# benabbouosama/DEEPL-Project

Measured on AMD Instinct MI355X. Metric: images/sec train step, TransVAE-Large f16d32 256px bs256, higher is better.
Workload: dtype bf16

## Files before the change

deepl-project_amd/csrc/conv3x3_halo.hip:

```cpp
#include "igemm_common.h"

namespace {

template <int BM, int BN, int WGM, int WGN, int BST, int EPI>
__global__ __launch_bounds__(WGM* WGN * 64) void conv3x3_halo_kernel(const IgemmArgs p) {
    constexpr int BK = 64, NW = WGM * WGN, TW = 16, TH = BM / TW, HWD = TW + 2, HP = (TH + 2) * HWD;
    constexpr int A_PIECES = (HP * 8 + 63) / 64;
    constexpr int WTM = BM / WGM, WTN = BN / WGN, MF = WTM / 16, NF = WTN / 16;
    constexpr bool PIPE_ALL = (MF + NF) * 4 * (BK / 32) <= (NW == 4 && BM == 256 ? 128 : 80);
    constexpr int A_IT = (A_PIECES + NW - 1) / NW;
    constexpr int A_BYTES = A_PIECES * 1024, B_BYTES = BN * BK * 2;
    constexpr int B_INSTR = BN / 8, B_IT = B_INSTR / NW;
    static_assert(BST == 2 || BST == 3, "weight ring depth");
    static_assert(B_INSTR % NW == 0 && WTM % 16 == 0 && WTN % 16 == 0, "tile shape");

    extern __shared__ __attribute__((aligned(16))) char smem[];
    TV_PROBE_DECL
    char* const a_buf = smem;
    char* const b_buf = smem + 2 * A_BYTES;

    const int tid = threadIdx.x;
    const int lane = tid & 63;
    const int wave = __builtin_amdgcn_readfirstlane(tid >> 6);
    const int wm = wave / WGN, wn = wave % WGN;
    int tile_n, tile_m;
    if (p.xcd_order) {
        const int lin = blockIdx.x, j = lin >> 3;
        tile_n = j % p.tiles_n;
        tile_m = (j / p.tiles_n) * 8 + (lin & 7);
        if (tile_m >= p.tiles_m) return;
    } else {
        tile_n = blockIdx.x % p.tiles_n;
        tile_m = blockIdx.x / p.tiles_n;
    }
    const int n0 = tile_n * BN;
    const int tiles_x = p.w_out / TW, tiles_y = p.h_out / TH;
    const int b = tile_m / (tiles_x * tiles_y);
    const int trem = tile_m - b * (tiles_x * tiles_y);
    const int y0 = (trem / tiles_x) * TH, x0 = (trem % tiles_x) * TW;

    const int a_c16 = ((lane & 7) ^ ((lane >> 3) & 7)) * 16;
    auto a_voff_of = [&](int j) {
        int l8 = lane >> 3;
        asm volatile("" : "+v"(l8));
        const int hp = j * 8 + l8;
        const int hy = hp / HWD, hx = hp - hy * HWD;
        const int iy = y0 - 1 + hy, ix = x0 - 1 + hx;
        const bool ok = hp < HP && (unsigned)iy < (unsigned)p.h_in && (unsigned)ix < (unsigned)p.w_in;
        return ok ? ((b * p.h_in + iy) * p.w_in + ix) * p.ldx * 2 + a_c16 : OOB_OFFSET;
    };
    auto b_voff_of = [&](int j) {
        int l8 = lane >> 3;
        asm volatile("" : "+v"(l8));
        const int row = j * 8 + l8;
        const int rl = row % WTN;
        const int fr = bfrag_reader(rl);
        const int c = ((lane & 7) ^ swz_of<BK>(fr)) * 8;
        const int n = n0 + row;
        return (n < p.N) ? (n * p.K + c) * 2 : OOB_OFFSET;
    };
#ifdef TV_ABL_K1
    const int cch = 1;
#else
    const int cch = p.c_in / BK;
#endif

    constexpr bool VOFF_REGS = MF * NF * 4 + (MF + NF) * 8 <= 160 || BST == 3 || !PIPE_ALL;
    int a_voff_r[VOFF_REGS ? A_IT : 1], b_voff_r[VOFF_REGS ? B_IT : 1];
    if constexpr (VOFF_REGS) {
#pragma unroll
        for (int it = 0; it < A_IT; ++it) a_voff_r[it] = a_voff_of(it * NW + wave);
#pragma unroll
// ... 61 lines not shown
                        acc[i][j] = __builtin_amdgcn_mfma_f32_16x16x32_bf16(bfr[kk][j], af[kk][i], acc[i][j], 0, 0, 0);
                        const int idx = (kk * MF + i) * NF + j;
                        if (idx % GAP == GAP - 1 && idx / GAP < NIH) {
                            __builtin_amdgcn_sched_barrier(0);
                            issue(idx / GAP);
                            __builtin_amdgcn_sched_barrier(0);
                        }
                    }
        } else {
#pragma unroll
            for (int kk = 0; kk < BK / 32; ++kk) {
                bf16x8 af[MF], bfr[NF];
#pragma unroll
                for (int i = 0; i < MF; ++i) af[i] = *(const bf16x8*)(abase + a_off[i] + (((kk * 4 + fq) ^ a_sw[i]) << 4));
                const int coff = ((kk * 4 + fq) ^ sw) * 16;
#pragma unroll
                for (int j = 0; j < NF; ++j) bfr[j] = *(const bf16x8*)(bbase + b_row_off + bfrag_off(j) * (BK * 2) + coff);
#pragma unroll
                for (int i = 0; i < MF; ++i)
#pragma unroll
                    for (int j = 0; j < NF; ++j) {
                        acc[i][j] = __builtin_amdgcn_mfma_f32_16x16x32_bf16(bfr[j], af[i], acc[i][j], 0, 0, 0);
                        const int idx = (kk * MF + i) * NF + j;
                        if (idx % GAP == GAP - 1 && idx / GAP < NIH) {
                            __builtin_amdgcn_sched_barrier(0);
                            issue(idx / GAP);
                            __builtin_amdgcn_sched_barrier(0);
                        }
                    }
            }
        }
    };

    constexpr bool PP = NW == 8 && PIPE_ALL && BST == 3;
    if constexpr (PP) {
        constexpr int ATAPS = 6, A_PT = (A_IT + ATAPS - 1) / ATAPS;
        static_assert(A_PT == 1, "one halo piece per wave and tap");
        constexpr auto nsure = [](int tap) { return (tap >= 0 && tap < ATAPS && tap < A_IT && (tap + 1) * NW <= A_PIECES) ? 1 : 0; };
        const int grp = wave >> 2;
        bf16x8 fa[2][MF], fb[2][NF];
#pragma unroll
        for (int it = 0; it < A_IT; ++it) issue_a(a_buf, it, 0);
        issue_b(b_buf, 0, 0);
        issue_b(b_buf + B_BYTES, 1, 0);
        wait_vmcnt<0>();
        if (grp == 1) __builtin_amdgcn_s_barrier();
        int bcur = 0;
        for (int ch = 0; ch < cch; ++ch) {
            const char* acur = a_buf + (ch & 1) * A_BYTES;
            char* anxt = a_buf + ((ch + 1) & 1) * A_BYTES;
            const bool more = ch + 1 < cch;
            static_for<9>([&](auto tap_c) {
                constexpr int tap = decltype(tap_c)::value;
                constexpr int toff = (tap / 3) * HWD + (tap % 3);
                const char* const bslot = b_buf + bcur * B_BYTES;
                char* const bfill = b_buf + ((bcur + 2 >= BST) ? bcur + 2 - BST : bcur + 2) * B_BYTES;
                const bool b_go = (tap + 2 < 9) || more;
                const int b_koff = ((tap + 2 < 9) ? (tap + 2) * p.c_in + ch * BK : (tap + 2 - 9) * p.c_in + (ch + 1) * BK) * 2;
                auto load_dma = [&]() {
                    if (b_go) {
#pragma unroll
                        for (int it = 0; it < B_IT; ++it) issue_b_piece(bfill, it, b_koff);
                    }
                    if (tap < ATAPS && tap < A_IT && more) issue_a(anxt, tap, ch + 1);
                };
                __builtin_amdgcn_s_barrier();
                TV_T(1);
                int hpb = hp_base;
                asm volatile("" : "+v"(hpb));
#ifndef TV_ABL_NO_LDSREAD
#pragma unroll
                for (int kk = 0; kk < 2; ++kk) {
#pragma unroll
                    for (int i = 0; i < MF; ++i) {
                        const int hp = hpb + i * HWD + toff;
                        fa[kk][i] = *(const bf16x8*)(acur + hp * (BK * 2) + (((kk * 4 + fq) ^ (hp & 7)) << 4));
                    }
                    const int coff = ((kk * 4 + fq) ^ sw) * 16;
#pragma unroll
                    for (int j = 0; j < NF; ++j) fb[kk][j] = *(const bf16x8*)(bslot + b_row_off + bfrag_off(j) * (BK * 2) + coff);
                }
#else
                if (tap == 0 && ch == 0) {
                    for (int kk = 0; kk < 2; ++kk) {
                        for (int i = 0; i < MF; ++i) { fa[kk][i] = bf16x8{1, 1, 1, 1, 1, 1, 1, 1}; asm volatile("" : "+v"(fa[kk][i])); }
                        for (int j = 0; j < NF; ++j) { fb[kk][j] = bf16x8{1, 1, 1, 1, 1, 1, 1, 1}; asm volatile("" : "+v"(fb[kk][j])); }
                    }
                }
#endif
                __builtin_amdgcn_sched_barrier(0);
                TV_T(3);
                load_dma();
                __builtin_amdgcn_sched_barrier(0);
                TV_T(2);
                asm volatile("s_waitcnt lgkmcnt(0)" ::: "memory");
                if (more) wait_vmcnt<nsure(tap - 1) + B_IT + nsure(tap)>();
                else if (tap + 2 < 9) wait_vmcnt<B_IT>();
                else wait_vmcnt<0>();
                TV_T(0);
                __builtin_amdgcn_s_barrier();
                TV_T(5);
                __builtin_amdgcn_s_setprio(1);
#pragma unroll
                for (int kk = 0; kk < 2; ++kk)
#pragma unroll
                    for (int i = 0; i < MF; ++i)
#pragma unroll
                        for (int j = 0; j < NF; ++j) acc[i][j] = __builtin_amdgcn_mfma_f32_16x16x32_bf16(fb[kk][j], fa[kk][i], acc[i][j], 0, 0, 0);
                __builtin_amdgcn_s_setprio(0);
                __builtin_amdgcn_sched_barrier(0);
                TV_T(4);
                bcur = (bcur + 1 == BST) ? 0 : bcur + 1;
            });
        }
        if (grp == 0) __builtin_amdgcn_s_barrier();
    } else if constexpr (PIPE_ALL) {
        constexpr int ATAPS = 6, A_PT = (A_IT + ATAPS - 1) / ATAPS;
        constexpr auto nsure = [](int tap) {
            int n = 0;
            for (int it = tap * A_PT; it < tap * A_PT + A_PT; ++it)
                if (tap >= 0 && tap < ATAPS && it < A_IT && (it + 1) * NW <= A_PIECES) ++n;
            return n;
        };
        constexpr int HMF = MF * NF, NIS = B_IT + A_PT, HGAP = HMF / NIS;
        static_assert(HGAP >= 1, "more DMA pieces than MFMAs in a half-step");
        bf16x8 f0a[MF], f0b[NF], f1a[MF], f1b[NF];
#ifdef TV_ABL_CHEAP_ADDR
        const int abl_a_off = (hp_base & ~7) * (BK * 2) + fi * (BK * 2) + ((fq ^ (fi & 7)) << 4);
#endif
#ifdef TV_ABL_NO_LDSREAD
        for (int i = 0; i < MF; ++i) { f0a[i] = bf16x8{1, 1, 1, 1, 1, 1, 1, 1}; f1a[i] = f0a[i]; asm volatile("" : "+v"(f0a[i]), "+v"(f1a[i])); }
        for (int j = 0; j < NF; ++j) { f0b[j] = bf16x8{1, 1, 1, 1, 1, 1, 1, 1}; f1b[j] = f0b[j]; asm volatile("" : "+v"(f0b[j]), "+v"(f1b[j])); }
#endif
        auto read_half = [&](const char* abase, const char* bbase, int toff, int kk, bf16x8 (&fa)[MF], bf16x8 (&fb)[NF]) {
#ifdef TV_ABL_NO_LDSREAD
            return;
#endif
            int hpb = hp_base;
            asm volatile("" : "+v"(hpb));
#pragma unroll
            for (int i = 0; i < MF; ++i) {
#ifdef TV_ABL_CHEAP_ADDR
                fa[i] = *(const bf16x8*)(abase + abl_a_off + i * HWD * (BK * 2) + kk * 64);
#else
                const int hp = hpb + i * HWD + toff;
                fa[i] = *(const bf16x8*)(abase + hp * (BK * 2) + (((kk * 4 + fq) ^ (hp & 7)) << 4));
#endif
            }
// ... 144 lines not shown
    __builtin_amdgcn_s_setprio(0);
    TV_T(5);
#ifdef TV_ABL_NO_EPI
    {
        float chk = 0.f;
#pragma unroll
        for (int i = 0; i < MF; ++i)
#pragma unroll
            for (int j = 0; j < NF; ++j) chk += acc[i][j][0] + acc[i][j][1] + acc[i][j][2] + acc[i][j][3];
        if (chk != 123.456f) return;
    }
#endif
    f32x4 bvals[NF];
    load_bias<WTN>(p, lane, n0 + wn * WTN, bvals);
    const int pix0 = (b * p.h_out + y0 + wm * MF) * p.w_out + x0;
    epilogue<WTM, WTN, EPI, true>(p, acc, bvals, smem, wave, lane, n0 + wn * WTN, [&](int r) { return pix0 + (r >> 4) * p.w_out + (r & 15); });
    TV_T(6);
    TV_PROBE_DUMP(wave, lane);
}

template <int BM, int BN, int WGM, int WGN, int BST>
int launch_halo_one(const IgemmArgs& a_in, hipStream_t s) {
    constexpr int NW = WGM * WGN, HP = (BM / 16 + 2) * 18;
    constexpr int RING = 2 * (((HP * 8 + 63) / 64) * 1024) + BST * BN * 64 * 2;
    constexpr int EPI = epilogue_lds_bytes<BM / WGM, BN / WGN>(NW);
    constexpr int BYTES = RING > EPI ? RING : EPI;
    if constexpr (BYTES > LDS_MAX) {
        return -1;
    } else {
        const int tiles_m = a_in.batch * (a_in.h_out / (BM / 16)) * (a_in.w_out / 16);
        IgemmArgs a = a_in;
        a.tiles_m = tiles_m;
        a.xcd_order = (g_xcd_order && a.tiles_n > 1) ? 1 : 0;
        dim3 grid((unsigned)(a.xcd_order ? 8 * a.tiles_n * ((tiles_m + 7) / 8) : tiles_m * a.tiles_n)), block(NW * 64);
        auto go = [&](auto epi) {
            constexpr int EPI_MODE = decltype(epi)::value;
            static TvPerDeviceOnce attr_once;
            if (attr_once.first()) {
                (void)hipFuncSetAttribute((const void*)conv3x3_halo_kernel<BM, BN, WGM, WGN, BST, EPI_MODE>, hipFuncAttributeMaxDynamicSharedMemorySize, BYTES);
            }
            hipLaunchKernelGGL((conv3x3_halo_kernel<BM, BN, WGM, WGN, BST, EPI_MODE>), grid, block, BYTES, s, a);
        };
        const int epi = epilogue_mode(a);
        if (epi == 1) go(std::integral_constant<int, 1>{});
        else if (epi == 2) go(std::integral_constant<int, 2>{});
        else go(std::integral_constant<int, 0>{});
        return 0;
    }
}

template <int BM, int BN, int WGM, int WGN>
int launch_halo_ring(const IgemmArgs& a, int ring, hipStream_t s) {
    if (ring >= 3 && launch_halo_one<BM, BN, WGM, WGN, 3>(a, s) == 0) return 0;
    return launch_halo_one<BM, BN, WGM, WGN, 2>(a, s);
}

int launch_halo_impl(IgemmArgs& a, hipStream_t s) {
    if (!(a.kh == 3 && a.kw == 3 && a.stride == 1 && a.pad == 1 && a.up_shift == 0 && a.dil_mask == 0 && !a.shuffle)) return -1;
    if (a.c_in % 64 != 0 || a.N <= 64 || a.x_bytes == 0 || a.w_bytes == 0) return -1;
    if (a.h_in != a.h_out || a.w_in != a.w_out || a.w_out % 16 != 0 || a.h_out % 8 != 0) return -1;
    const int N = a.N;
    const bool h16 = a.h_out % 16 == 0;
    int bm = 128;
    int bn = pick_tile(a.M, N, h16, h16 && (N == 192 || N % 128 != 0), &bm);
    if (N % 192 == 0 && h16 && g_cfg_bn == 0 && g_halo_ring == 3 && !g_halo_w4) { bn = 192; bm = 256; }
    if (g_cfg_bn == 256 && N % 256 == 0 && h16) { bn = 256; bm = 256; }
    else if (g_cfg_bn == 192 && N % 192 == 0 && h16) { bn = 192; bm = 256; }
    else if (g_cfg_bn == 128) { bn = (N % 192 == 0 && N % 128 != 0) ? 192 : 128; bm = 128; }
    if (g_cfg_bm) bm = g_cfg_bm;
    if (bm == 256 && !h16) bm = 128;
    if (bn == 192) {
        a.tiles_n = N / 192;
        if (bm == 256 && g_halo_w4) return launch_halo_ring<256, 192, 2, 2>(a, (g_halo_ring == 3 && a.tiles_n == 1) || g_halo_ring == 4 ? 3 : 2, s);
        if (bm == 256) return launch_halo_ring<256, 192, 4, 2>(a, (g_halo_ring == 3 || g_halo_ring == 4) ? 3 : 2, s);
        return launch_halo_ring<128, 192, 2, 2>(a, g_halo_ring == 4 ? 3 : 2, s);
    }
// ... 18 lines not shown
```

deepl-project_amd/csrc/igemm_common.h:

```cpp
#pragma once
#pragma clang fp contract(off)
#include "common.h"

#include <type_traits>

namespace tvi {

struct IgemmArgs {
    const bf16* x;
    const bf16* w;
    const float* bias;
    const bf16* res;
    const bf16* aux;
    bf16* pre;
    bf16* out;
    const char* zeros;
    int M, N, K;
    int batch, h_in, w_in, c_in, ldx;
    int h_out, w_out, ldo;
    int kh, kw, stride, pad, up_shift, dil_mask;
    int tiles_n, tiles_m, xcd_order;
    int sup_r, sup_c;
    int tpb, nchunks;
    int shuffle;
    int act;
    int aux_act;
    int pre_deriv;
    int form;
    const float* rope;
    int rope_tokens, rope_cols;
    int hw_shift, w_shift;
    unsigned dv_hw_m, dv_w_m, dv_cq_m;
    int dv_hw_s, dv_w_s, dv_cq_s;
    int store_nt;
    unsigned out_bytes;
    unsigned x_bytes, w_bytes;
    const bf16* x2;
    unsigned x2_bytes;
    int ldx2, k1_steps;
};

constexpr int LDS_MAX = 160 * 1024;
extern int g_cfg_bm, g_cfg_bn, g_halo_ring;
extern bool g_halo_w4, g_xcd_order, g_epi_modes;
int epilogue_mode(const IgemmArgs& a);
int pick_tile(long long M, int N, bool allow256, bool allow192_256rows, int* bm);
int launch_halo(IgemmArgs& a, hipStream_t s);
#ifdef TV_PROBE
int set_halo_probe(void* dev_buf);
#endif

}

namespace {
using namespace tvi;

#ifndef TV_PIPE_ALL_MAX
#define TV_PIPE_ALL_MAX 80
#endif
#ifndef TV_RD_THREAD
#define TV_RD_THREAD 0
#endif
#ifndef TV_GENERIC_DPHASE
#define TV_GENERIC_DPHASE 1
#endif
#ifndef TV_PERSIST_DRAIN
#define TV_PERSIST_DRAIN 1
#endif

__device__ __forceinline__ constexpr int bfrag_off(int j) { return (j >> 1) * 32 + (j & 1) * 4; }
__device__ __forceinline__ int bfrag_lane_row(int fi) { return (fi >> 2) * 8 + (fi & 3); }
__device__ __forceinline__ int bfrag_reader(int rl) { return (((rl & 31) >> 3) << 2) | (rl & 3); }

__device__ __forceinline__ int fast_div(int x, unsigned m, int sh) {
    return m ? (int)(__umulhi((unsigned)x, m) >> sh) : x;
}
// ... 539 lines not shown
```

deepl-project_amd/csrc/igemm_nt.hip:

```cpp
#include "igemm_common.h"

namespace tvi {
int g_cfg_bm = 0;
int g_cfg_bn = 0;
int g_halo_ring = 3;
bool g_halo_w4 = false;
bool g_xcd_order = true;
int g_supertile = 0;
bool g_epi_modes = true;

int epilogue_mode(const IgemmArgs& a) {
    if (a.rope) return 0;
    if (!g_epi_modes || a.shuffle || a.pre || a.out_bytes == 0) return 0;
    if (a.aux) return (a.aux_act == TV_ACT_DERIV && !a.res) ? 2 : 0;
    return (a.res && a.act == TV_ACT_NONE) ? 1 : 0;
}

int pick_tile(long long M, int N, bool allow256, bool allow192_256rows, int* bm) {
    const long long m256 = (M + 255) / 256, m128 = (M + 127) / 128;
    double best = 1e30;
    int bn = 128;
    *bm = 128;
    auto consider = [&](int cbn, int cbm, long long tiles, double slots, double eff) {
        const double rounds = (double)((long long)((tiles + slots - 1) / slots));
        const double t = rounds * (double)cbm * cbn * (slots / 256.0) / eff;
        if (t < best) { best = t; bn = cbn; *bm = cbm; }
    };
    consider(128, 128, m128 * ((N + 127) / 128), 512.0, 0.85);
    if (N % 192 == 0 && allow192_256rows) consider(192, 256, m256 * (N / 192), 256.0, 0.97);
    if (N % 192 == 0 && N % 128 != 0) consider(192, 128, m128 * (N / 192), 256.0, 0.80);
    if (N % 256 == 0 && allow256) consider(256, 256, m256 * (N / 256), 256.0, 1.0);
    return bn;
}

}

namespace {

// ... 850 lines not shown
    return launch_mode<BK, 1>(a, s);
}

}

extern "C" int tv_set_dma(int on) {
    g_use_dma = on != 0;
    g_addr_mode = (on == 2) ? 1 : 0;
    return 0;
}

extern "C" int tv_set_igemm_halo(int on) {
    g_halo_w4 = on >= 100;
    on %= 100;
    g_xcd_order = on < 10;
    on %= 10;
    g_use_halo = on != 0;
    g_halo_ring = (on == 2) ? 2 : (on == 4 ? 4 : 3);
    return 0;
}

extern "C" int tv_set_igemm_nt_threshold(int mib) {
    g_nt_threshold_mb = mib;
    return 0;
}

extern "C" int tv_set_igemm_persist(int on) {
    if (on == -1) g_loop8 = 0;
    else if (on == -2) g_loop8 = 1;
    else g_persist = on;
    return 0;
}

extern "C" int tv_set_igemm_supertile(int v) {
    g_supertile = v;
    return 0;
}

extern "C" int tv_set_igemm_epilogue(int on) {
    g_epi_modes = on != 0;
    return 0;
}

#ifdef TV_PROBE
extern "C" int tv_set_igemm_probe(void* dev_buf) {
    const bool ok = hipMemcpyToSymbol(HIP_SYMBOL(g_probe_dev), &dev_buf, sizeof(void*)) == hipSuccess;
    return (tvi::set_halo_probe(dev_buf) == 0 && ok) ? 0 : 1;
}
#endif

extern "C" int tv_set_igemm_config(int bm, int bn, int stages, int bk) {
    g_cfg_bm = bm;
    g_cfg_bn = bn;
    g_cfg_stages = stages;
    g_cfg_bk = bk;
    return 0;
}

struct RopeSpec {
    const float* tab;
    int tokens, cols;
};
struct Cat2Spec {
    const void* x2;
    int k1, ldx2;
};
// ... 138 lines not shown
```

deepl-project_amd/transvae/hip/_lib.py:

```python
from __future__ import annotations

import ctypes as C
import glob
import os
import subprocess
import threading

_HERE = os.path.dirname(os.path.abspath(__file__))
PKG_ROOT = os.path.dirname(os.path.dirname(_HERE))
CSRC = os.path.join(PKG_ROOT, "csrc")
SO_PATH = os.environ.get("TV_HIP_SO") or os.path.join(_HERE, "libtransvae_hip.so")

ACT_NONE, ACT_GELU, ACT_SILU = 0, 1, 2
ACT_DERIV, ACT_SAVE_DERIV = 3, 16
ACT_ADD = 4
ACTX_RELU = 5
ACTX_LRELU = 6
GAN_GEN, GAN_BCE, GAN_HINGE, GAN_WGAN = 0, 1, 2, 3
LPIPS_MAP, LPIPS_SIGMOID, LPIPS_CLAMP = 1, 2, 4
POOL3_MAX_S2, POOL3_MAX_S1P1, POOL3_AVG_S1P1 = 0, 1, 2
SSIM_SKIMAGE, SSIM_BOX11 = 0, 1
METRIC_NONE, METRIC_CLIP, METRIC_SIGMOID = 0, 1, 2
IMAGE_NONE, IMAGE_SIGMOID = 0, 1
ERR_UNSUPPORTED = 4
# ... 171 lines not shown
    if r.returncode != 0:
        raise RuntimeError(f"link failed:\n{r.stdout.decode(errors='replace')}")
    return SO_PATH


def load():
    global _lib
    if _lib is not None:
        return _lib
    with _lock:
        if _lib is not None:
            return _lib
        if not os.path.exists(SO_PATH):
            raise RuntimeError(
                f"{SO_PATH} is missing: build it with `python -c 'import __graft_entry__ as g; g.build()'` "
                "(the TransVAE path has no non-HIP fallback)")
        lib = C.CDLL(SO_PATH)
        for name, (res, args) in SIGNATURES.items():
            fn = getattr(lib, name)
            fn.restype = res
            fn.argtypes = args
        lib.tv_set_dma.restype = _I
        lib.tv_set_dma.argtypes = [_I]
        lib.tv_set_igemm_halo.restype = _I
        lib.tv_set_igemm_halo.argtypes = [_I]
        lib.tv_set_igemm_epilogue.restype = _I
        lib.tv_set_igemm_epilogue.argtypes = [_I]
        lib.tv_set_igemm_nt_threshold.restype = _I
        lib.tv_set_igemm_nt_threshold.argtypes = [_I]
        if os.environ.get("TV_IGEMM_NT_MB") is not None:
            lib.tv_set_igemm_nt_threshold(int(os.environ["TV_IGEMM_NT_MB"]))
        lib.tv_set_igemm_persist.restype = _I
        lib.tv_set_igemm_persist.argtypes = [_I]
        lib.tv_set_attn_bwd_mask.restype = _I
        lib.tv_set_attn_bwd_mask.argtypes = [_I]
        lib.tv_set_igemm_config.restype = _I
        lib.tv_set_igemm_config.argtypes = [_I, _I, _I, _I]
        lib.tv_set_wgrad_stages.restype = _I
        lib.tv_set_wgrad_stages.argtypes = [_I]
        lib.tv_set_wgrad_config.restype = _I
        lib.tv_set_wgrad_config.argtypes = [_I, _I, _I]
        lib.tv_set_wgrad_kx3.restype = _I
        lib.tv_set_wgrad_kx3.argtypes = [_I, _I, _I]
        lib.tv_wgrad_tn_which.restype = _I
        lib.tv_wgrad_tn_which.argtypes = [_DP, _I, _I, _I, C.c_char_p, _I]
        if os.environ.get("TV_WGRAD_KX3") is not None:
            lib.tv_set_wgrad_kx3(int(os.environ["TV_WGRAD_KX3"]), 0, 0)
        _lib = lib
    return _lib


def check(rc: int, what: str = "") -> None:
    if rc != 0:
        msg = load().tv_last_error().decode(errors="replace")
        raise RuntimeError(f"libtransvae_hip {what} failed (status {rc}): {msg}")
```

deepl-project_amd/csrc/attention.hip:

```cpp
#include "common.h"

namespace {

#ifndef TV_ATTN_ABL
#define TV_ATTN_ABL 0
#endif
__device__ __forceinline__ f32x16 mfma32(bf16x8 a, bf16x8 b, f32x16 c) {
#if TV_ATTN_ABL & 4
    c[0] += (float)a[0] * (float)b[0];
    return c;
#else
    return __builtin_amdgcn_mfma_f32_32x32x16_bf16(a, b, c, 0, 0, 0);
#endif
}
__device__ __forceinline__ f32x16 mfma32b(bf16x8 a, bf16x8 b, f32x16 c) {
#if TV_ATTN_ABL & 2
    c[0] += (float)a[0] * (float)b[0];
    return c;
#else
    return __builtin_amdgcn_mfma_f32_32x32x16_bf16(a, b, c, 0, 0, 0);
#endif
}
#if TV_ATTN_ABL & 1
__device__ __forceinline__ float fexp2(float x) { return x; }
// ... 635 lines not shown
            const bf16x8 df = pack_acc(s, ss);
#pragma unroll
            for (int db = 0; db < 2; ++db) dqt[db] = mfma32b(kfr[ss][db], df, dqt[db]);
        }
    };
    auto key_block = [&](int t, auto stage_c) {
        constexpr int S = decltype(stage_c)::value;
        if (t + D - 1 < nblk) vm_wait<PIECES * (D - 1)>();
        else vm_wait<0>();
        block_sync();
        half_block(t, stage_c, ic<0>{});
        half_block(t, stage_c, ic<1>{});
    };
    ring_for<NS>(nblk, key_block);
    if (q_ok) {
        bf16* row = p.out + ((size_t)b * p.N + qi) * ld + head * 64;
#pragma unroll
        for (int db = 0; db < 2; ++db)
#pragma unroll
            for (int g = 0; g < 4; ++g) {
                float f[4] = {dqt[db][4 * g] * p.scale, dqt[db][4 * g + 1] * p.scale, dqt[db][4 * g + 2] * p.scale, dqt[db][4 * g + 3] * p.scale};
                if (p.rope) rope_adjoint4(f, p.rope + (size_t)qi * 128, db * 32 + 8 * g + 4 * h);
                bf16x4 v = {(bf16)f[0], (bf16)f[1], (bf16)f[2], (bf16)f[3]};
                attn_store4(row + db * 32 + 8 * g + 4 * h, v);
            }
    }
}

#ifndef TV_ATTN_DKV_QS
#define TV_ATTN_DKV_QS 2
#endif
constexpr int DKV_QS = TV_ATTN_DKV_QS;
constexpr int QT_TILE = DKV_QS * 32 * 128;
constexpr int DKV_STAGE = 2 * QT_TILE + DKV_QS * 256;

__global__ __launch_bounds__(256) void attn_bwd_dkv_kernel(const AttnArgs p) {
    extern __shared__ __attribute__((aligned(16))) char smem[];
    const int lane = threadIdx.x & 63;
    const int wave = __builtin_amdgcn_readfirstlane(threadIdx.x >> 6);
    int tile_x, head, b;
    if (!attn_block(p, tile_x, head, b)) return;
    const int C = p.heads * 64;
    const size_t ld = (size_t)3 * C;
    const bf16* qbase = p.qkv + (size_t)b * p.N * ld + head * 64;
    const bf16* kbase = qbase + C;
    const bf16* vbase = qbase + 2 * C;
    const bf16* gbase = p.d_o + (size_t)b * p.N * C + head * 64;
    const float* del_b = p.delta + ((size_t)b * p.heads + head) * p.N;
    const float* lse_b = del_b + (size_t)p.B * p.heads * p.N;
    const int k0 = tile_x * 128 + wave * 32;
    const int ki = k0 + (lane & 31);
    const int h = lane >> 5;
    const bool k_ok = ki < p.N;

    bf16x8 kf[4], vf[4];
#pragma unroll
    for (int st = 0; st < 4; ++st) {
        bf16x8 a = {0, 0, 0, 0, 0, 0, 0, 0}, v = {0, 0, 0, 0, 0, 0, 0, 0};
        if (k_ok) {
            a = *(const bf16x8*)(kbase + (size_t)ki * ld + 16 * st + 8 * h);
            v = *(const bf16x8*)(vbase + (size_t)ki * ld + 16 * st + 8 * h);
        }
        kf[st] = a;
        vf[st] = v;
    }
    f32x16 dkt[2], dvt[2];
#pragma unroll
    for (int i = 0; i < 16; ++i) dkt[0][i] = dkt[1][i] = dvt[0][i] = dvt[1][i] = 0.f;
    const float c2 = p.scale * 1.4426950408889634f;
    const int ntile = (p.N + 32 * DKV_QS - 1) / (32 * DKV_QS);
    int off_r[4], off_c[2], off_ch[2];
    rows_offsets(lane, off_r);
    cols_offsets<false>(lane, off_c, off_ch);

    int vo_q[DKV_QS], vo_g[DKV_QS];
    stage_offsets<false>(vo_q, (int)ld, wave, lane);
    stage_offsets<false>(vo_g, C, wave, lane);
    const unsigned q_bytes = stage_extent(p.N, (int)ld), g_bytes = stage_extent(p.N, C);
    auto stage = [&](int t, char* sb) {
        stage_rows_buf(sb, qbase, q_bytes, t * 32 * DKV_QS, (int)ld, vo_q, wave);
        stage_rows_buf(sb + QT_TILE, gbase, g_bytes, t * 32 * DKV_QS, C, vo_g, wave);
        if (wave < DKV_QS) {
            const int q = (t * DKV_QS + wave) * 32 + (lane & 31);
            const float* src = (q < p.N) ? ((lane < 32 ? lse_b : del_b) + q) : (const float*)(p.zeros + lane * 4);
            __builtin_amdgcn_global_load_lds(TV_GLB(src), TV_LDS(sb + 2 * QT_TILE + wave * 256), 4, 0, 0);
        }
    };

    const unsigned smem_addr = (unsigned)(uintptr_t)(__attribute__((address_space(3))) char*)smem;
    const char* abs_r[4];
    unsigned abs_c[2], abs_ch[2];
#pragma unroll
    for (int st = 0; st < 4; ++st) abs_r[st] = smem + off_r[st];
#pragma unroll
    for (int db = 0; db < 2; ++db) {
        abs_c[db] = smem_addr + off_c[db];
        abs_ch[db] = smem_addr + off_ch[db];
    }
    const char* abs_st = smem + 16 * h;
    constexpr int NS = TV_ATTN_NS_DKV, D = NS - 1;
#pragma unroll
    for (int i = 0; i < D; ++i)
        if (i < ntile) stage(i, smem + i * DKV_STAGE);
    auto query_tile = [&](int t, auto stage_c, auto sub_c) {
        constexpr int S = decltype(stage_c)::value, U = decltype(sub_c)::value;
        constexpr int QB = S * DKV_STAGE + U * 32 * 128, GB = QB + QT_TILE;
        constexpr int STB = S * DKV_STAGE + 2 * QT_TILE + U * 256;
        f32x16 s, dp;
#pragma unroll
        for (int i = 0; i < 16; ++i) s[i] = 0.f;
        f32x4 nl[4], nd[4];
        nl[0] = *(const f32x4*)(abs_st + STB + 0);
        nl[1] = *(const f32x4*)(abs_st + STB + 32);
        nl[2] = *(const f32x4*)(abs_st + STB + 64);
        nl[3] = *(const f32x4*)(abs_st + STB + 96);
        nd[0] = *(const f32x4*)(abs_st + STB + 128 + 0);
        nd[1] = *(const f32x4*)(abs_st + STB + 128 + 32);
        nd[2] = *(const f32x4*)(abs_st + STB + 128 + 64);
        nd[3] = *(const f32x4*)(abs_st + STB + 128 + 96);
#pragma unroll
        for (int r = 0; r < 16; ++r) dp[r] = nd[r >> 2][r & 3];
        s = mfma32(read_rows_imm<QB>(abs_r[0]), kf[0], s);
        dp = mfma32(read_rows_imm<GB>(abs_r[0]), vf[0], dp);
        s = mfma32(read_rows_imm<QB>(abs_r[1]), kf[1], s);
        dp = mfma32(read_rows_imm<GB>(abs_r[1]), vf[1], dp);
        s = mfma32(read_rows_imm<QB>(abs_r[2]), kf[2], s);
        dp = mfma32(read_rows_imm<GB>(abs_r[2]), vf[2], dp);
        s = mfma32(read_rows_imm<QB>(abs_r[3]), kf[3], s);
        dp = mfma32(read_rows_imm<GB>(abs_r[3]), vf[3], dp);
        if constexpr (U == 0) {
            __builtin_amdgcn_sched_barrier(0);
            if (!(TV_ATTN_ABL & 8) && t + D < ntile) stage(t + D, smem + ((S + D) % NS) * DKV_STAGE);
            __builtin_amdgcn_sched_barrier(0);
        }
        bf16x8 gfr[2][2], qfr[2][2];
#pragma unroll
        for (int db = 0; db < 2; ++db) {
            gfr[0][db] = read_cols_imm<GB>(abs_c[db], abs_ch[db]);
            gfr[1][db] = read_cols_imm<GB + 16 * 128>(abs_c[db], abs_ch[db]);
            qfr[0][db] = read_cols_imm<QB>(abs_c[db], abs_ch[db]);
            qfr[1][db] = read_cols_imm<QB + 16 * 128>(abs_c[db], abs_ch[db]);
        }
#pragma unroll
        for (int r = 0; r < 16; ++r) {
            const float pv = fexp2(fmaf(s[r], c2, nl[r >> 2][r & 3]));
            s[r] = pv;
            dp[r] = pv * dp[r];
        }
        lds_wait_all();
#pragma unroll
        for (int ss = 0; ss < 2; ++ss) {
            const bf16x8 pf = pack_acc(s, ss);
            const bf16x8 df = pack_acc(dp, ss);
#pragma unroll
            for (int db = 0; db < 2; ++db) {
                dvt[db] = mfma32b(gfr[ss][db], pf, dvt[db]);
                dkt[db] = mfma32b(qfr[ss][db], df, dkt[db]);
            }
        }
    };
    auto query_stage = [&](int t, auto stage_c) {
        constexpr int S = decltype(stage_c)::value;
        if (t + D - 1 < ntile) {
            if (wave < DKV_QS) vm_wait<(2 * DKV_QS + 1) * (D - 1)>();
            else vm_wait<2 * DKV_QS * (D - 1)>();
        } else {
            vm_wait<0>();
        }
        block_sync();
        query_tile(t, stage_c, ic<0>{});
        if constexpr (DKV_QS > 1) {
            if ((t * DKV_QS + 1) * 32 < p.N) query_tile(t, stage_c, ic<1>{});
        }
    };
    ring_for<NS>(ntile, query_stage);
    if (k_ok) {
        bf16* krow = p.out + ((size_t)b * p.N + ki) * ld + C + head * 64;
        bf16* vrow = krow + C;
#pragma unroll
        for (int db = 0; db < 2; ++db)
#pragma unroll
            for (int g = 0; g < 4; ++g) {
                float f[4] = {dkt[db][4 * g] * p.scale, dkt[db][4 * g + 1] * p.scale, dkt[db][4 * g + 2] * p.scale, dkt[db][4 * g + 3] * p.scale};
                if (p.rope) rope_adjoint4(f, p.rope + (size_t)ki * 128, db * 32 + 8 * g + 4 * h);
                bf16x4 a = {(bf16)f[0], (bf16)f[1], (bf16)f[2], (bf16)f[3]};
                bf16x4 v = {(bf16)dvt[db][4 * g], (bf16)dvt[db][4 * g + 1], (bf16)dvt[db][4 * g + 2], (bf16)dvt[db][4 * g + 3]};
                attn_store4(krow + db * 32 + 8 * g + 4 * h, a);
                attn_store4(vrow + db * 32 + 8 * g + 4 * h, v);
            }
    }
}

int attn_check(const char* name, int B, int N, int heads, float scale) {
    if (B <= 0 || N <= 0 || heads <= 0 || !(scale > 0.f) || B > 65535 || heads > 65535) {
        tv_set_error("%s: bad shape B=%d N=%d heads=%d scale=%g", name, B, N, heads, (double)scale);
        return TV_ERR_ARG;
    }
    return TV_OK;
}

}

static int g_attn_bwd_mask = 7;
extern "C" int tv_set_attn_bwd_mask(int mask) {
    g_attn_bwd_mask = mask;
// ... 48 lines not shown
```

Before: 160.2.

## Let halo conv3x3 blocks walk several consecutive M tiles with overlapped prefetch

In the pipelined 8-wave halo conv kernel, each block now processes a run of consecutive output tiles (walk) instead of one. The next tile's halo and weight loads are issued during the current tile's last channel chunk, so loads overlap the epilogue, and the vmcnt waits are relaxed to account for the epilogue's outstanding stores. A host heuristic picks walk from tile count versus a 256-slot wave model, and it can be overridden with a new setter. This removes per-block prologue and fill bubbles, at the cost of longer runs that may hurt load balance and of more complex synchronization and register pressure.

```diff
diff --git a/deepl-project_amd/csrc/conv3x3_halo.hip b/deepl-project_amd/csrc/conv3x3_halo.hip
--- a/deepl-project_amd/csrc/conv3x3_halo.hip
+++ b/deepl-project_amd/csrc/conv3x3_halo.hip
@@ -23,21 +23,23 @@
     const int lane = tid & 63;
     const int wave = __builtin_amdgcn_readfirstlane(tid >> 6);
     const int wm = wave / WGN, wn = wave % WGN;
+    constexpr bool PP = NW == 8 && PIPE_ALL && BST == 3;
+    const int walk = PP ? p.walk : 1;
     int tile_n, tile_m;
     if (p.xcd_order) {
         const int lin = blockIdx.x, j = lin >> 3;
         tile_n = j % p.tiles_n;
-        tile_m = (j / p.tiles_n) * 8 + (lin & 7);
+        tile_m = ((j / p.tiles_n) * 8 + (lin & 7)) * walk;
         if (tile_m >= p.tiles_m) return;
     } else {
         tile_n = blockIdx.x % p.tiles_n;
-        tile_m = blockIdx.x / p.tiles_n;
+        tile_m = (blockIdx.x / p.tiles_n) * walk;
     }
     const int n0 = tile_n * BN;
     const int tiles_x = p.w_out / TW, tiles_y = p.h_out / TH;
-    const int b = tile_m / (tiles_x * tiles_y);
+    int b = tile_m / (tiles_x * tiles_y);
     const int trem = tile_m - b * (tiles_x * tiles_y);
-    const int y0 = (trem / tiles_x) * TH, x0 = (trem % tiles_x) * TW;
+    int y0 = (trem / tiles_x) * TH, x0 = (trem % tiles_x) * TW;
 
     const int a_c16 = ((lane & 7) ^ ((lane >> 3) & 7)) * 16;
     auto a_voff_of = [&](int j) {
@@ -165,37 +167,56 @@
         }
     };
 
-    constexpr bool PP = NW == 8 && PIPE_ALL && BST == 3;
     if constexpr (PP) {
         constexpr int ATAPS = 6, A_PT = (A_IT + ATAPS - 1) / ATAPS;
         static_assert(A_PT == 1, "one halo piece per wave and tap");
         constexpr auto nsure = [](int tap) { return (tap >= 0 && tap < ATAPS && tap < A_IT && (tap + 1) * NW <= A_PIECES) ? 1 : 0; };
+        constexpr int NST = MF * (NF / 2);
         const int grp = wave >> 2;
         bf16x8 fa[2][MF], fb[2][NF];
+        const int tile_end = tile_m + walk < p.tiles_m ? tile_m + walk : p.tiles_m;
+        constexpr bool BIAS_RUN = EPI != 0;
+        f32x4 bvals[NF];
+        if constexpr (BIAS_RUN) load_bias<WTN>(p, lane, n0 + wn * WTN, bvals);
 #pragma unroll
         for (int it = 0; it < A_IT; ++it) issue_a(a_buf, it, 0);
         issue_b(b_buf, 0, 0);
         issue_b(b_buf + B_BYTES, 1, 0);
         wait_vmcnt<0>();
         if (grp == 1) __builtin_amdgcn_s_barrier();
-        int bcur = 0;
-        for (int ch = 0; ch < cch; ++ch) {
-            const char* acur = a_buf + (ch & 1) * A_BYTES;
-            char* anxt = a_buf + ((ch + 1) & 1) * A_BYTES;
-            const bool more = ch + 1 < cch;
+        int bcur = 0, apar = 0;
+        int pix0 = (b * p.h_out + y0 + wm * MF) * p.w_out + x0;
+#pragma nounroll
+        for (int ch = 0, tm = tile_m;;) {
+            const bool next = tm + 1 < tile_end, later = tm != tile_m;
+            const char* acur = a_buf + apar * A_BYTES;
+            char* anxt = a_buf + (apar ^ 1) * A_BYTES;
+            apar ^= 1;
+            const bool last = ch + 1 == cch;
+            const bool more = !last || next;
+            const int chn = last ? 0 : ch + 1;
+            if (last && next) {
+                x0 += TW;
+                if (x0 == p.w_out) { x0 = 0; y0 += TH; }
+                if (y0 == p.h_out) { y0 = 0; ++b; }
+                if constexpr (VOFF_REGS) {
+#pragma unroll
+                    for (int it = 0; it < A_IT; ++it) a_voff_r[it] = a_voff_of(it * NW + wave);
+                }
+            }
             static_for<9>([&](auto tap_c) {
                 constexpr int tap = decltype(tap_c)::value;
                 constexpr int toff = (tap / 3) * HWD + (tap % 3);
                 const char* const bslot = b_buf + bcur * B_BYTES;
                 char* const bfill = b_buf + ((bcur + 2 >= BST) ? bcur + 2 - BST : bcur + 2) * B_BYTES;
                 const bool b_go = (tap + 2 < 9) || more;
-                const int b_koff = ((tap + 2 < 9) ? (tap + 2) * p.c_in + ch * BK : (tap + 2 - 9) * p.c_in + (ch + 1) * BK) * 2;
+                const int b_koff = ((tap + 2 < 9) ? (tap + 2) * p.c_in + ch * BK : (tap + 2 - 9) * p.c_in + chn * BK) * 2;
                 auto load_dma = [&]() {
                     if (b_go) {
 #pragma unroll
                         for (int it = 0; it < B_IT; ++it) issue_b_piece(bfill, it, b_koff);
                     }
-                    if (tap < ATAPS && tap < A_IT && more) issue_a(anxt, tap, ch + 1);
+                    if (tap < ATAPS && tap < A_IT && more) issue_a(anxt, tap, chn);
                 };
                 __builtin_amdgcn_s_barrier();
                 TV_T(1);
@@ -227,8 +248,22 @@
                 __builtin_amdgcn_sched_barrier(0);
                 TV_T(2);
                 asm volatile("s_waitcnt lgkmcnt(0)" ::: "memory");
-                if (more) wait_vmcnt<nsure(tap - 1) + B_IT + nsure(tap)>();
-                else if (tap + 2 < 9) wait_vmcnt<B_IT>();
+                auto wait_more = [&](auto base_c) {
+                    constexpr int BASE = decltype(base_c)::value;
+#ifndef TV_ABL_WALK_DRAIN
+                    if constexpr (tap == 0) {
+                        static_assert(BASE + 2 * NST <= 63, "vmcnt is a 6-bit count");
+                        if (ch == 0 && later) {
+                            if (EPI == 0 && (p.form == EF_GELU_D || p.form == EF_SILU_D)) wait_vmcnt<BASE + 2 * NST>();
+                            else wait_vmcnt<BASE + NST>();
+                            return;
+                        }
+                    }
+#endif
+                    wait_vmcnt<BASE>();
+                };
+                if (more) wait_more(std::integral_constant<int, nsure(tap - 1) + B_IT + nsure(tap)>{});
+                else if (tap + 2 < 9) wait_more(std::integral_constant<int, B_IT>{});
                 else wait_vmcnt<0>();
                 TV_T(0);
                 __builtin_amdgcn_s_barrier();
@@ -245,8 +280,44 @@
                 TV_T(4);
                 bcur = (bcur + 1 == BST) ? 0 : bcur + 1;
             });
+            if (!last) {
+                ++ch;
+                continue;
+            }
+            if (grp == 0) __builtin_amdgcn_s_barrier();
+            __builtin_amdgcn_s_setprio(0);
+            TV_T(5);
+            int lane_e = lane;
+            asm volatile("" : "+v"(lane_e));
+            IgemmArgs pe = p;
+            asm volatile("" : "+s"(pe.out), "+s"(pe.pre), "+s"(pe.res), "+s"(pe.aux), "+s"(pe.out_bytes), "+s"(pe.M), "+s"(pe.N), "+s"(pe.ldo),
+                         "+s"(pe.form), "+s"(pe.store_nt), "+s"(pe.bias));
+            if constexpr (!BIAS_RUN) load_bias<WTN>(pe, lane_e, n0 + wn * WTN, bvals);
+#ifdef TV_ABL_NO_EPI
+            float chk = 0.f;
+#pragma unroll
+            for (int i = 0; i < MF; ++i)
+#pragma unroll
+                for (int j = 0; j < NF; ++j) chk += acc[i][j][0] + acc[i][j][1] + acc[i][j][2] + acc[i][j][3];
+            if (chk == 123.456f)
+#endif
+            epilogue<WTM, WTN, EPI, true>(pe, acc, bvals, smem, wave, lane_e, n0 + wn * WTN, [&](int r) { return pix0 + (r >> 4) * p.w_out + (r & 15); });
+            TV_T(6);
+            if (!next) break;
+#pragma unroll
+            for (int i = 0; i < MF; ++i)
+#pragma unroll
+                for (int j = 0; j < NF; ++j) acc[i][j] = f32x4{0.f, 0.f, 0.f, 0.f};
+#ifdef TV_ABL_WALK_DRAIN
+            wait_vmcnt<0>();
+#endif
+            if (grp == 1) __builtin_amdgcn_s_barrier();
+            ch = 0;
+            ++tm;
+            pix0 = (b * p.h_out + y0 + wm * MF) * p.w_out + x0;
         }
-        if (grp == 0) __builtin_amdgcn_s_barrier();
+        TV_PROBE_DUMP(wave, lane);
+        return;
     } else if constexpr (PIPE_ALL) {
         constexpr int ATAPS = 6, A_PT = (A_IT + ATAPS - 1) / ATAPS;
         constexpr auto nsure = [](int tap) {
@@ -457,7 +528,30 @@
         IgemmArgs a = a_in;
         a.tiles_m = tiles_m;
         a.xcd_order = (g_xcd_order && a.tiles_n > 1) ? 1 : 0;
-        dim3 grid((unsigned)(a.xcd_order ? 8 * a.tiles_n * ((tiles_m + 7) / 8) : tiles_m * a.tiles_n)), block(NW * 64);
+        const int epi = epilogue_mode(a);
+        a.walk = 1;
+        constexpr bool WALK_OK = BM == 256 && BN == 192 && NW == 8 && BST == 3;
+        auto direct_form = [](int f) {
+            switch (f) {
+                case EF_PLAIN: case EF_GELU_D: case EF_SILU_D: case EF_GELU: case EF_SILU: case EF_RES_DERIV: case EF_RES2:
+                case EF_RELU: case EF_RELU_MASK: case EF_LRELU: case EF_LRELU_MASK: return true;
+                default: return false;
+            }
+        };
+        if (WALK_OK && g_halo_walk != 1 && (epi != 0 || direct_form(a.form))) {
+            if (g_halo_walk > 1) {
+                a.walk = g_halo_walk < tiles_m ? g_halo_walk : tiles_m;
+            } else {
+                long long best = 0;
+                for (int w = 1; w <= 16; w *= 2) {
+                    const long long runs = (long long)((tiles_m + w - 1) / w) * a.tiles_n;
+                    const long long cost = ((runs + 255) / 256) * (12 * w + 1);
+                    if (w == 1 || cost < best) { best = cost; a.walk = w; }
+                }
+            }
+        }
+        const int runs_m = (tiles_m + a.walk - 1) / a.walk;
+        dim3 grid((unsigned)(a.xcd_order ? 8 * a.tiles_n * ((runs_m + 7) / 8) : runs_m * a.tiles_n)), block(NW * 64);
         auto go = [&](auto epi) {
             constexpr int EPI_MODE = decltype(epi)::value;
             static TvPerDeviceOnce attr_once;
@@ -466,7 +560,6 @@
             }
             hipLaunchKernelGGL((conv3x3_halo_kernel<BM, BN, WGM, WGN, BST, EPI_MODE>), grid, block, BYTES, s, a);
         };
-        const int epi = epilogue_mode(a);
         if (epi == 1) go(std::integral_constant<int, 1>{});
         else if (epi == 2) go(std::integral_constant<int, 2>{});
         else go(std::integral_constant<int, 0>{});
diff --git a/deepl-project_amd/csrc/igemm_common.h b/deepl-project_amd/csrc/igemm_common.h
--- a/deepl-project_amd/csrc/igemm_common.h
+++ b/deepl-project_amd/csrc/igemm_common.h
@@ -22,6 +22,7 @@
     int tiles_n, tiles_m, xcd_order;
     int sup_r, sup_c;
     int tpb, nchunks;
+    int walk;
     int shuffle;
     int act;
     int aux_act;
@@ -41,7 +42,7 @@
 };
 
 constexpr int LDS_MAX = 160 * 1024;
-extern int g_cfg_bm, g_cfg_bn, g_halo_ring;
+extern int g_cfg_bm, g_cfg_bn, g_halo_ring, g_halo_walk;
 extern bool g_halo_w4, g_xcd_order, g_epi_modes;
 int epilogue_mode(const IgemmArgs& a);
 int pick_tile(long long M, int N, bool allow256, bool allow192_256rows, int* bm);
diff --git a/deepl-project_amd/csrc/igemm_nt.hip b/deepl-project_amd/csrc/igemm_nt.hip
--- a/deepl-project_amd/csrc/igemm_nt.hip
+++ b/deepl-project_amd/csrc/igemm_nt.hip
@@ -4,6 +4,7 @@
 int g_cfg_bm = 0;
 int g_cfg_bn = 0;
 int g_halo_ring = 3;
+int g_halo_walk = 0;
 bool g_halo_w4 = false;
 bool g_xcd_order = true;
 int g_supertile = 0;
@@ -920,6 +921,11 @@
     return 0;
 }
 
+extern "C" int tv_set_halo_walk(int n) {
+    g_halo_walk = n < 0 ? 0 : n;
+    return 0;
+}
+
 extern "C" int tv_set_igemm_supertile(int v) {
     g_supertile = v;
     return 0;
diff --git a/deepl-project_amd/transvae/hip/_lib.py b/deepl-project_amd/transvae/hip/_lib.py
--- a/deepl-project_amd/transvae/hip/_lib.py
+++ b/deepl-project_amd/transvae/hip/_lib.py
@@ -227,6 +227,8 @@
             lib.tv_set_igemm_nt_threshold(int(os.environ["TV_IGEMM_NT_MB"]))
         lib.tv_set_igemm_persist.restype = _I
         lib.tv_set_igemm_persist.argtypes = [_I]
+        lib.tv_set_halo_walk.restype = _I
+        lib.tv_set_halo_walk.argtypes = [_I]
         lib.tv_set_attn_bwd_mask.restype = _I
         lib.tv_set_attn_bwd_mask.argtypes = [_I]
         lib.tv_set_igemm_config.restype = _I
```

New measurement: 160.1. About the same (-0.0%).

## Restructure attention dK/dV backward tile loop with staged LDS reads and occupancy hint

Applied to the files above, without the earlier changes.

Splits the dK/dV backward query-tile body into score, softmax and accumulate phases. It software-pipelines the row-fragment LDS reads two steps ahead of the MFMAs and waits on each half's column fragments separately instead of one global lgkmcnt wait. The LSE/delta statistics load becomes a single buffer load per wave with hardware bounds clamping, replacing per-lane pointer selection against a zeros buffer, and the stats layout changes to one 64-float row per stage. It also adds a launch-bounds occupancy hint of 3. Risks include register pressure from the occupancy target and a hard assumption that DKV_QS is 2.

```diff
diff --git a/deepl-project_amd/csrc/attention.hip b/deepl-project_amd/csrc/attention.hip
--- a/deepl-project_amd/csrc/attention.hip
+++ b/deepl-project_amd/csrc/attention.hip
@@ -691,9 +691,16 @@
 #endif
 constexpr int DKV_QS = TV_ATTN_DKV_QS;
 constexpr int QT_TILE = DKV_QS * 32 * 128;
-constexpr int DKV_STAGE = 2 * QT_TILE + DKV_QS * 256;
-
-__global__ __launch_bounds__(256) void attn_bwd_dkv_kernel(const AttnArgs p) {
+constexpr int DKV_STAGE = 2 * QT_TILE + 512;
+static_assert(DKV_QS == 2, "a statistics row of 64 floats covers the two 32-query tiles of a ring stage");
+#ifndef TV_ATTN_DKV_OCC
+#define TV_ATTN_DKV_OCC 3
+#endif
+__device__ __forceinline__ void lds_wait_frags(bf16x8& a, bf16x8& b, bf16x8& c, bf16x8& d) {
+    asm volatile("s_waitcnt lgkmcnt(0)" : "+v"(a), "+v"(b), "+v"(c), "+v"(d)::"memory");
+}
+
+__global__ __launch_bounds__(256, TV_ATTN_DKV_OCC) void attn_bwd_dkv_kernel(const AttnArgs p) {
     extern __shared__ __attribute__((aligned(16))) char smem[];
     const int lane = threadIdx.x & 63;
     const int wave = __builtin_amdgcn_readfirstlane(threadIdx.x >> 6);
@@ -739,10 +746,11 @@
     auto stage = [&](int t, char* sb) {
         stage_rows_buf(sb, qbase, q_bytes, t * 32 * DKV_QS, (int)ld, vo_q, wave);
         stage_rows_buf(sb + QT_TILE, gbase, g_bytes, t * 32 * DKV_QS, C, vo_g, wave);
-        if (wave < DKV_QS) {
-            const int q = (t * DKV_QS + wave) * 32 + (lane & 31);
-            const float* src = (q < p.N) ? ((lane < 32 ? lse_b : del_b) + q) : (const float*)(p.zeros + lane * 4);
-            __builtin_amdgcn_global_load_lds(TV_GLB(src), TV_LDS(sb + 2 * QT_TILE + wave * 256), 4, 0, 0);
+        if (wave < 2) {
+#if defined(__HIP_DEVICE_COMPILE__)
+            __builtin_amdgcn_raw_ptr_buffer_load_lds(__builtin_amdgcn_make_buffer_rsrc(const_cast<float*>(wave == 0 ? lse_b : del_b), 0, p.N * 4, 0x00020000),
+                                                     TV_LDS(sb + 2 * QT_TILE + wave * 256), 4, lane * 4, t * 256, 0, 0);
+#endif
         }
     };
 
@@ -761,62 +769,85 @@
 #pragma unroll
     for (int i = 0; i < D; ++i)
         if (i < ntile) stage(i, smem + i * DKV_STAGE);
-    auto query_tile = [&](int t, auto stage_c, auto sub_c) {
+    auto tile_scores = [&](auto stage_c, auto sub_c, f32x16& s, f32x16& dp) {
         constexpr int S = decltype(stage_c)::value, U = decltype(sub_c)::value;
         constexpr int QB = S * DKV_STAGE + U * 32 * 128, GB = QB + QT_TILE;
-        constexpr int STB = S * DKV_STAGE + 2 * QT_TILE + U * 256;
+        constexpr int STD = S * DKV_STAGE + 2 * QT_TILE + 256 + U * 128;
+#pragma unroll
+        for (int i = 0; i < 16; ++i) s[i] = 0.f;
+#pragma unroll
+        for (int g = 0; g < 4; ++g) {
+            const f32x4 nd = *(const f32x4*)(abs_st + STD + 32 * g);
+#pragma unroll
+            for (int e = 0; e < 4; ++e) dp[4 * g + e] = nd[e];
+        }
+        bf16x8 rq[4], rg[4];
+        rq[0] = read_rows_imm<QB>(abs_r[0]);
+        rg[0] = read_rows_imm<GB>(abs_r[0]);
+        rq[1] = read_rows_imm<QB>(abs_r[1]);
+        rg[1] = read_rows_imm<GB>(abs_r[1]);
+        __builtin_amdgcn_sched_barrier(0);
+#pragma unroll
+        for (int i = 0; i < 4; ++i) {
+            if (i + 2 < 4) {
+                rq[i + 2] = read_rows_imm<QB>(abs_r[i + 2]);
+                rg[i + 2] = read_rows_imm<GB>(abs_r[i + 2]);
+            }
+            s = mfma32(rq[i], kf[i], s);
+            dp = mfma32(rg[i], vf[i], dp);
+            __builtin_amdgcn_sched_barrier(0);
+        }
+    };
+    auto softmax4 = [&](const f32x4& nl, int g, f32x16& s, f32x16& dp) {
+#pragma unroll
+        for (int e = 0; e < 4; ++e) {
+            const float pv = fexp2(fmaf(s[4 * g + e], c2, nl[e]));
+            s[4 * g + e] = pv;
+            dp[4 * g + e] = pv * dp[4 * g + e];
+        }
+    };
+    auto tile_softmax = [&](auto stage_c, auto sub_c, f32x16& s, f32x16& dp) {
+        constexpr int STB = decltype(stage_c)::value * DKV_STAGE + 2 * QT_TILE + decltype(sub_c)::value * 128;
+#pragma unroll
+        for (int g = 0; g < 4; ++g) softmax4(*(const f32x4*)(abs_st + STB + 32 * g), g, s, dp);
+    };
+    auto read_frags = [&](auto stage_c, auto sub_c, auto ss_c, bf16x8 (&gq)[4]) {
+        constexpr int QB = decltype(stage_c)::value * DKV_STAGE + decltype(sub_c)::value * 32 * 128 + decltype(ss_c)::value * 16 * 128;
+        constexpr int GB = QB + QT_TILE;
+        gq[0] = read_cols_imm<GB>(abs_c[0], abs_ch[0]);
+        gq[1] = read_cols_imm<QB>(abs_c[0], abs_ch[0]);
+        gq[2] = read_cols_imm<GB>(abs_c[1], abs_ch[1]);
+        gq[3] = read_cols_imm<QB>(abs_c[1], abs_ch[1]);
+    };
+    auto accum_half = [&](const bf16x8 (&gq)[4], const bf16x8& pf, const bf16x8& df) {
+        dvt[0] = mfma32b(gq[0], pf, dvt[0]);
+        dkt[0] = mfma32b(gq[1], df, dkt[0]);
+        dvt[1] = mfma32b(gq[2], pf, dvt[1]);
+        dkt[1] = mfma32b(gq[3], df, dkt[1]);
+    };
+    auto tile_accum = [&](auto stage_c, auto sub_c, const f32x16& s, const f32x16& dp) {
+        bf16x8 f0[4], f1[4];
+        read_frags(stage_c, sub_c, ic<0>{}, f0);
+        const bf16x8 pf0 = pack_acc(s, 0), df0 = pack_acc(dp, 0);
+        lds_wait_frags(f0[0], f0[1], f0[2], f0[3]);
+        read_frags(stage_c, sub_c, ic<1>{}, f1);
+        accum_half(f0, pf0, df0);
+        const bf16x8 pf1 = pack_acc(s, 1), df1 = pack_acc(dp, 1);
+        lds_wait_frags(f1[0], f1[1], f1[2], f1[3]);
+        accum_half(f1, pf1, df1);
+    };
+    auto stage_next = [&](int t, auto stage_c) {
+        constexpr int S = decltype(stage_c)::value;
+        __builtin_amdgcn_sched_barrier(0);
+        if (!(TV_ATTN_ABL & 8) && t + D < ntile) stage(t + D, smem + ((S + D) % NS) * DKV_STAGE);
+        __builtin_amdgcn_sched_barrier(0);
+    };
+    auto tile_serial = [&](int t, auto stage_c, auto sub_c) {
         f32x16 s, dp;
-#pragma unroll
-        for (int i = 0; i < 16; ++i) s[i] = 0.f;
-        f32x4 nl[4], nd[4];
-        nl[0] = *(const f32x4*)(abs_st + STB + 0);
-        nl[1] = *(const f32x4*)(abs_st + STB + 32);
-        nl[2] = *(const f32x4*)(abs_st + STB + 64);
-        nl[3] = *(const f32x4*)(abs_st + STB + 96);
-        nd[0] = *(const f32x4*)(abs_st + STB + 128 + 0);
-        nd[1] = *(const f32x4*)(abs_st + STB + 128 + 32);
-        nd[2] = *(const f32x4*)(abs_st + STB + 128 + 64);
-        nd[3] = *(const f32x4*)(abs_st + STB + 128 + 96);
-#pragma unroll
-        for (int r = 0; r < 16; ++r) dp[r] = nd[r >> 2][r & 3];
-        s = mfma32(read_rows_imm<QB>(abs_r[0]), kf[0], s);
-        dp = mfma32(read_rows_imm<GB>(abs_r[0]), vf[0], dp);
-        s = mfma32(read_rows_imm<QB>(abs_r[1]), kf[1], s);
-        dp = mfma32(read_rows_imm<GB>(abs_r[1]), vf[1], dp);
-        s = mfma32(read_rows_imm<QB>(abs_r[2]), kf[2], s);
-        dp = mfma32(read_rows_imm<GB>(abs_r[2]), vf[2], dp);
-        s = mfma32(read_rows_imm<QB>(abs_r[3]), kf[3], s);
-        dp = mfma32(read_rows_imm<GB>(abs_r[3]), vf[3], dp);
-        if constexpr (U == 0) {
-            __builtin_amdgcn_sched_barrier(0);
-            if (!(TV_ATTN_ABL & 8) && t + D < ntile) stage(t + D, smem + ((S + D) % NS) * DKV_STAGE);
-            __builtin_amdgcn_sched_barrier(0);
-        }
-        bf16x8 gfr[2][2], qfr[2][2];
-#pragma unroll
-        for (int db = 0; db < 2; ++db) {
-            gfr[0][db] = read_cols_imm<GB>(abs_c[db], abs_ch[db]);
-            gfr[1][db] = read_cols_imm<GB + 16 * 128>(abs_c[db], abs_ch[db]);
-            qfr[0][db] = read_cols_imm<QB>(abs_c[db], abs_ch[db]);
-            qfr[1][db] = read_cols_imm<QB + 16 * 128>(abs_c[db], abs_ch[db]);
-        }
-#pragma unroll
-        for (int r = 0; r < 16; ++r) {
-            const float pv = fexp2(fmaf(s[r], c2, nl[r >> 2][r & 3]));
-            s[r] = pv;
-            dp[r] = pv * dp[r];
-        }
-        lds_wait_all();
-#pragma unroll
-        for (int ss = 0; ss < 2; ++ss) {
-            const bf16x8 pf = pack_acc(s, ss);
-            const bf16x8 df = pack_acc(dp, ss);
-#pragma unroll
-            for (int db = 0; db < 2; ++db) {
-                dvt[db] = mfma32b(gfr[ss][db], pf, dvt[db]);
-                dkt[db] = mfma32b(qfr[ss][db], df, dkt[db]);
-            }
-        }
+        tile_scores(stage_c, sub_c, s, dp);
+        if constexpr (decltype(sub_c)::value == 0) stage_next(t, stage_c);
+        tile_softmax(stage_c, sub_c, s, dp);
+        tile_accum(stage_c, sub_c, s, dp);
     };
     auto query_stage = [&](int t, auto stage_c) {
         constexpr int S = decltype(stage_c)::value;
@@ -827,9 +858,9 @@
             vm_wait<0>();
         }
         block_sync();
-        query_tile(t, stage_c, ic<0>{});
+        tile_serial(t, stage_c, ic<0>{});
         if constexpr (DKV_QS > 1) {
-            if ((t * DKV_QS + 1) * 32 < p.N) query_tile(t, stage_c, ic<1>{});
+            if ((t * DKV_QS + 1) * 32 < p.N) tile_serial(t, stage_c, ic<1>{});
         }
     };
     ring_for<NS>(ntile, query_stage);
```

After: 160.7 before, 161.5 after (median of 6 runs). Within noise of the previous version (+0.5%).
